# cr1m5onk1ng/text_similarity

Hardware: AMD Instinct MI355X
Metric: sentences/sec encoded + Mpairs/sec cosine top-k @ N=1M d=384 (higher is better)
Workload: dtype bf16 encoder / f16 selection / fp32 scores

## Files before the change

text_similarity_amd/csrc/encoder.hip:

```cpp
#include <math.h>
#include <cmath>

#include <stdlib.h>
#include <string.h>

#include <vector>

#include <type_traits>
#include <utility>

#include "common.h"
#include "gemm_pp.h"

namespace tsim {

__device__ __forceinline__ int64_t packed_off(int64_t t, int f, int W) {
    return ((t >> 5) * (W >> 3) + (f >> 3)) * 256 + (t & 31) * 8 + (f & 7);
}

template <int VPL, bool TYPED = false>
__global__ __launch_bounds__(256) void embed_ln_kernel(const int32_t *__restrict__ ids,
                                                       const int32_t *__restrict__ pos,
                                                       const float *__restrict__ word,
                                                       const float *__restrict__ pos_emb,
// ... 1108 lines not shown
    if (wt) {
        const int i = lane & 15, g = lane >> 4;
        const int ntt = (d_out + 15) >> 4;
        const float *xp = x + (int64_t)min(r0 + i, B - 1) * d_in + 4 * g;
        const float *wp[NT];
#pragma unroll
        for (int t = 0; t < NT; ++t) wp[t] = wt + (int64_t)min((wv + DN_WAVES * t) * 16 + i, d_out - 1) * d_in + 4 * g;
        f32x4 acc[NT];
#pragma unroll
        for (int t = 0; t < NT; ++t) acc[t] = f32x4{0.f, 0.f, 0.f, 0.f};
        float4 a = load4_or_zero(xp, 4 * g < d_in), bw[NT];
#pragma unroll
        for (int t = 0; t < NT; ++t) bw[t] = load4_or_zero(wp[t], wv + DN_WAVES * t < ntt && 4 * g < d_in);
        for (int k0 = 0; k0 < d_in; k0 += 16) {
            const int k1 = k0 + 16;
            const bool kin = k1 + 4 * g < d_in;
            const float4 an = load4_or_zero(xp + k1, kin);
            float4 bn[NT];
#pragma unroll
            for (int t = 0; t < NT; ++t) bn[t] = load4_or_zero(wp[t] + k1, wv + DN_WAVES * t < ntt && kin);
#pragma unroll
            for (int t = 0; t < NT; ++t) {
                if (wv + DN_WAVES * t < ntt) {
                    acc[t] = __builtin_amdgcn_mfma_f32_16x16x4f32(a.x, bw[t].x, acc[t], 0, 0, 0);
                    acc[t] = __builtin_amdgcn_mfma_f32_16x16x4f32(a.y, bw[t].y, acc[t], 0, 0, 0);
                    acc[t] = __builtin_amdgcn_mfma_f32_16x16x4f32(a.z, bw[t].z, acc[t], 0, 0, 0);
                    acc[t] = __builtin_amdgcn_mfma_f32_16x16x4f32(a.w, bw[t].w, acc[t], 0, 0, 0);
                }
            }
            a = an;
#pragma unroll
            for (int t = 0; t < NT; ++t) bw[t] = bn[t];
        }
#pragma unroll
        for (int t = 0; t < NT; ++t) {
            const int col = (wv + DN_WAVES * t) * 16 + i;
            if (col < d_out) {
#pragma unroll
                for (int r = 0; r < 4; ++r) ys[(4 * g + r) * d_out + col] = acc[t][r];
            }
        }
    } else {
        for (int k = threadIdx.x; k < DN_ROWS * d_out; k += 64 * DN_WAVES) {
            const int r = k / d_out;
            ys[k] = r0 + r < B ? x[(int64_t)(r0 + r) * d_in + (k - r * d_out)] : 0.f;
        }
    }
    __syncthreads();
    for (int r = wv; r < DN_ROWS; r += DN_WAVES) {
        const int b = r0 + r;
        if (b >= B) break;
        float *y = ys + r * d_out;
        for (int j = lane; j < d_out; j += 64) {
            float v = y[j];
            if (bias) v += bias[j];
            if (act == TSIM_ACT_TANH) v = tanhf(v);
            y[j] = v;
        }
        if (normalize) {
            double ss = 0.0;
            for (int j = lane; j < d_out; j += 64) ss = fma((double)y[j], (double)y[j], ss);
            const double inv = canonical_inv_norm(ss, 1e-12f);
            for (int j = lane; j < d_out; j += 64) y[j] = canonical_scale_f32(y[j], inv);
        }
        if (out)
            for (int j = lane; j < d_out; j += 64) out[(int64_t)b * d_out + j] = y[j];
        if (unit) {
            double ss = 0.0;
            for (int j = lane; j < d_out; j += 64) ss = fma((double)y[j], (double)y[j], ss);
            const double inv = canonical_inv_norm(ss, 1e-8f);
            double r2 = 0.0;
            for (int j = lane; j < ld_unit; j += 64) {
                unit_t hv = (unit_t)0;
                if (j < d_out) {
                    hv = canonical_unit_elem(y[j], inv);
                    const double de = (double)(float)hv - (double)y[j] * inv;
                    r2 = fma(de, de, r2);
                }
                unit[(int64_t)b * ld_unit + j] = hv;
            }
            if (rho_max) {
                const float rho = rho_round_up(sqrt(wave_sum_f64(r2)));
                if (lane == 0) rho_publish(rho_max, rho);
            }
        }
    }
}

static int dense_rows_launch(const float *x, int B, int d_in, const float *w, const float *bias, int d_out, int act, int normalize,
                             float *out, unit_t *unit, int ld_unit, float *rho_max, hipStream_t st) {
    if (B <= 0) return TSIM_OK;
    const dim3 grid((unsigned)((B + DN_ROWS - 1) / DN_ROWS));
    const size_t lds = (size_t)DN_ROWS * d_out * sizeof(float);
#define DENSE(NT) hipLaunchKernelGGL(dense_rows_kernel<NT>, grid, dim3(64 * DN_WAVES), lds, st, x, B, d_in, w, bias, d_out, act, normalize, out, unit, ld_unit, rho_max)
    const int nt = ((d_out + 15) / 16 + DN_WAVES - 1) / DN_WAVES;
    if (nt <= 1) DENSE(1); else if (nt <= 2) DENSE(2); else if (nt <= 3) DENSE(3); else if (nt <= 4) DENSE(4);
    else if (nt <= 6) DENSE(6); else DENSE(8);
#undef DENSE
    TSIM_HIP_CHECK(hipGetLastError());
    return TSIM_OK;
}

static int dense_check(int d_in, int d_out, int act, const float *w) {
    TSIM_REQUIRE(d_in >= 8 && d_in <= DN_MAX && d_in % 8 == 0, "dense: d_in=%d outside [8, %d] or not a multiple of 8", d_in, DN_MAX);
    TSIM_REQUIRE(d_out >= 8 && d_out <= DN_MAX && d_out % 8 == 0, "dense: d_out=%d outside [8, %d] or not a multiple of 8", d_out,
                 DN_MAX);
    TSIM_REQUIRE(w || d_out == d_in, "dense: without a weight matrix d_out (%d) must equal d_in (%d)", d_out, d_in);
    TSIM_REQUIRE(act == TSIM_ACT_IDENTITY || act == TSIM_ACT_TANH, "dense: unknown activation %d (TSIM_ACT_IDENTITY, TSIM_ACT_TANH)",
                 act);
    TSIM_REQUIRE(((uintptr_t)w & 15) == 0, "dense: the weight matrix must be 16-byte aligned");
    return TSIM_OK;
}

static uint16_t host_f32_to_bf16(float f) {
    uint32_t u;
    memcpy(&u, &f, 4);
    if ((u & 0x7fffffffu) > 0x7f800000u) return (uint16_t)((u >> 16) | 0x40);
    u += 0x7fffu + ((u >> 16) & 1u);
    return (uint16_t)(u >> 16);
}

struct DevBuf {
    void *p = nullptr;
    ~DevBuf() {
        if (p) (void)hipFree(p);
    }
};

}

using namespace tsim;

struct tsim_encoder {
    tsim_encoder_config cfg;
    int Tp = 0;
    float *word = nullptr, *pos = nullptr, *type0 = nullptr, *emb_g = nullptr, *emb_b = nullptr, *relb = nullptr;
    int relw = 0;
    int n_types = 0;
    float *head_wpT = nullptr, *head_bp = nullptr, *head_wc = nullptr, *head_bc = nullptr;
    int n_labels = 0;
    struct Layer {
        bf16_t *wqkv, *wo, *w1, *w2;
        bf16_t *pqkv = nullptr, *po = nullptr;
        bf16_t *lo = nullptr, *l2 = nullptr;
        bf16_t *lo32 = nullptr, *l232 = nullptr;
        uint8_t *qqkv = nullptr, *qo = nullptr, *q1 = nullptr, *q2 = nullptr;
        uint8_t *sqkv = nullptr, *so = nullptr, *s1 = nullptr, *s2 = nullptr;
        float *bqkv, *bo, *b1, *b2, *g1, *be1, *g2, *be2;
    };
    std::vector<Layer> layers;
    std::vector<void *> allocs;
    bf16_t *x0 = nullptr, *x1 = nullptr, *qkv = nullptr, *ctx = nullptr, *h1 = nullptr;
    float *ybuf = nullptr;
    float *head_x = nullptr;
    uint8_t *aq = nullptr, *as = nullptr, *hq = nullptr, *hs = nullptr;
    int *err_flags = nullptr;
};

namespace tsim {

static int dev_alloc(tsim_encoder *e, size_t bytes, void **out) {
    void *p = nullptr;
    hipError_t err = hipMalloc(&p, bytes);
    if (err != hipSuccess) return fail(TSIM_ENOMEM, "hipMalloc(%zu) failed: %s", bytes, hipGetErrorString(err));
    e->allocs.push_back(p);
    *out = p;
    return TSIM_OK;
}

static int upload_f32(tsim_encoder *e, const float *h, size_t n, float **out) {
    int rc = dev_alloc(e, n * 4, (void **)out);
    if (rc) return rc;
    TSIM_HIP_CHECK(hipMemcpy(*out, h, n * 4, hipMemcpyHostToDevice));
    return TSIM_OK;
}

static int upload_bf16(tsim_encoder *e, const std::vector<const float *> &parts, size_t n_each, bf16_t **out) {
    std::vector<uint16_t> tmp(n_each * parts.size());
    for (size_t p = 0; p < parts.size(); ++p)
        for (size_t i = 0; i < n_each; ++i) tmp[p * n_each + i] = host_f32_to_bf16(parts[p][i]);
    int rc = dev_alloc(e, tmp.size() * 2, (void **)out);
    if (rc) return rc;
    TSIM_HIP_CHECK(hipMemcpy(*out, tmp.data(), tmp.size() * 2, hipMemcpyHostToDevice));
    return TSIM_OK;
}

static uint8_t host_f32_to_e4m3(float v) {
    const uint8_t sign = std::signbit(v) ? 0x80 : 0;
    const double a = std::fabs((double)v);
    if (a == 0.0) return sign;
    int exp;
    const double mant = std::frexp(a, &exp);
    long byte;
    if (a >= std::ldexp(1.0, -6))
        byte = ((long)(exp - 1 + 7) << 3) + std::lrint((mant * 2.0 - 1.0) * 8.0);
    else
        byte = std::lrint(std::ldexp(a, 9));
    if (byte > 0x7e) byte = 0x7e;
    return (uint8_t)byte | sign;
}

static int upload_mxfp8(tsim_encoder *e, const std::vector<const float *> &parts, size_t n_rows, size_t K, uint8_t **q,
                        uint8_t **sc) {
    const size_t rows = n_rows * parts.size(), nb = K / 32;
    std::vector<uint8_t> hq(rows * K), hs(rows * nb);
    for (size_t p = 0; p < parts.size(); ++p)
        for (size_t r = 0; r < n_rows; ++r)
            for (size_t b = 0; b < nb; ++b) {
                const float *src = parts[p] + r * K + b * 32;
                float amax = 0.f;
                for (int i = 0; i < 32; ++i) amax = std::fmax(amax, std::fabs(src[i]));
                int sexp = 0;
                if (amax > 0.f) {
                    int ex;
                    (void)std::frexp((double)amax, &ex);
                    sexp = ex - 1 - 8;
                    sexp = sexp < -127 ? -127 : (sexp > 127 ? 127 : sexp);
                }
                uint8_t *dst = hq.data() + (p * n_rows + r) * K + b * 32;
                for (int i = 0; i < 32; ++i) {
                    double y = std::ldexp((double)src[i], -sexp);
                    y = y > 448.0 ? 448.0 : (y < -448.0 ? -448.0 : y);
                    dst[i] = host_f32_to_e4m3((float)y);
                }
                hs[(p * n_rows + r) * nb + b] = (uint8_t)(sexp + 127);
            }
    int rc = dev_alloc(e, hq.size(), (void **)q);
    if (rc) return rc;
    if ((rc = dev_alloc(e, hs.size(), (void **)sc))) return rc;
    TSIM_HIP_CHECK(hipMemcpy(*q, hq.data(), hq.size(), hipMemcpyHostToDevice));
    TSIM_HIP_CHECK(hipMemcpy(*sc, hs.data(), hs.size(), hipMemcpyHostToDevice));
    return TSIM_OK;
}

static int mpnet_bucket(int rel, int num_buckets) {
    int ret = 0;
    int n = -rel;
    const int nb = num_buckets / 2;
    if (n < 0) {
        ret += nb;
        n = -n;
    }
    const int max_exact = nb / 2;
    if (n < max_exact) return ret + n;
    const float v = logf((float)n / (float)max_exact) / (float)log(128.0 / max_exact) * (float)(nb - max_exact);
    int large = max_exact + (int)v;
    if (large > nb - 1) large = nb - 1;
    return ret + large;
}

template <int BM, int BN, int BK, int WM, int WN, int EPI, int NST = 2>
static int launch_gemm(const bf16_t *X, const bf16_t *W, const float *bias, const bf16_t *res, const float *gamma,
                       const float *beta, float eps, bf16_t *out, int M, int N, int K, hipStream_t st,
                       const bf16_t *Wimg = nullptr, bool xpacked = false) {
    constexpr int lds = gemm_lds_bytes<BM, BN, BK, WM, WN, NST>();
    static_assert(lds <= 160 * 1024, "LDS budget");
    auto kern = gemm_bf16_kernel<BM, BN, BK, WM, WN, EPI, NST>;
    static DevOnce lds_once;
    TSIM_MAX_LDS(lds_once, kern, lds);
    if (N % BN != 0 || K % BK != 0) return fail(TSIM_EUNSUPPORTED, "gemm: N=%d K=%d not tileable by %dx%d", N, K, BN, BK);
    const int mtiles = (M + BM - 1) / BM, ntiles = N / BN;
    const int grid = ((mtiles + 7) / 8) * 8 * ntiles;
    if (Wimg && ntiles != 1) return fail(TSIM_EINVAL, "gemm: a packed W image needs BN == N");
    hipLaunchKernelGGL(kern, dim3(grid), dim3(WM * WN * 64), lds, st, X, W, bias, res, gamma, beta, eps, out, M, N, K,
                       mtiles, ntiles, Wimg, xpacked ? 1 : 0);
    TSIM_HIP_CHECK(hipGetLastError());
    return TSIM_OK;
}

template <int EPI, bool PK>
static int gemm_xres2(const bf16_t *X, const bf16_t *W, const float *bias, bf16_t *out, int M, int N, hipStream_t st) {
    constexpr int lds = X2_NSTAGE * X2_BN * X2_BK * 2 + 8192;
    if (N > 2048) return fail(TSIM_EUNSUPPORTED, "gemm_xres2: N=%d > 2048", N);
    if (((int64_t)M + 256) * N * 2 >= (1ll << 32)) return fail(TSIM_EUNSUPPORTED, "gemm_xres2: output of %d x %d exceeds 4 GiB", M, N);
    auto kern = gemm_xres2_kernel<EPI, PK>;
    static DevOnce lds_once;
    TSIM_MAX_LDS(lds_once, kern, lds);
    const int items = ((M + 255) / 256) * (N / X2_BN);
    const int grid = items < 256 ? items : 256;
    hipLaunchKernelGGL(kern, dim3(grid), dim3(512), lds, st, X, W, bias, out, M, N, items);
    TSIM_HIP_CHECK(hipGetLastError());
    return TSIM_OK;
}

typedef __attribute__((ext_vector_type(4))) uint32_t lt_u32x4;
constexpr int LT_PF = 12;
template <int PF>
__global__ __launch_bounds__(256) __attribute__((amdgpu_waves_per_eu(1, 1))) void ln_tail_gemm_kernel(
    const bf16_t *__restrict__ X, const bf16_t *__restrict__ Wimg32, const float *__restrict__ bias, const bf16_t *__restrict__ res,
    const float *__restrict__ gamma, const float *__restrict__ beta, float eps, bf16_t *__restrict__ out, int M, int K, int xpacked) {
    constexpr int N = 384, NT = 3, WAVES_N = 4, BM = 32;
    __shared__ float red[2 * WAVES_N * BM];
    const int lane = threadIdx.x & 63;
    const int wn = __builtin_amdgcn_readfirstlane(threadIdx.x >> 6);
    const int r = lane & 31, h = lane >> 5;
    const int m0 = blockIdx.x * BM;
    const int ksteps = K / 16;

    const int64_t mrow = (int64_t)(m0 + r < M ? m0 + r : M - 1);
    const char *xp = reinterpret_cast<const char *>(X) +
                     (xpacked ? (int64_t)(m0 >> 5) * K * 64 + h * 512 + r * 16
                              : (mrow * K + 8 * h) * 2);
    const int xstep = xpacked ? 1024 : 32;
    const char *wp = reinterpret_cast<const char *>(Wimg32) + (int64_t)(NT * wn) * 1024 + lane * 16;
    constexpr int WSTEP = (N / 32) * 1024;

    f32x16 acc[NT];
#pragma unroll
    for (int i = 0; i < NT; ++i)
#pragma unroll
        for (int gq = 0; gq < 4; ++gq) {
            const float4 bv = *reinterpret_cast<const float4 *>(bias + wn * 96 + 4 * h + i * 32 + 8 * gq);
            acc[i][4 * gq + 0] = bv.x;
            acc[i][4 * gq + 1] = bv.y;
            acc[i][4 * gq + 2] = bv.z;
            acc[i][4 * gq + 3] = bv.w;
        }
#pragma unroll
    for (int i = 0; i < NT; ++i) asm volatile("" : "+v"(acc[i]));

    lt_u32x4 fw[PF][NT], fx[PF];
    auto issue = [&](auto slotc, int s) __attribute__((always_inline)) {
        constexpr int slot = decltype(slotc)::value;
        const int sc = s < ksteps ? s : ksteps - 1;
        const char *w = wp + (int64_t)sc * WSTEP;
        const char *x = xp + (int64_t)sc * xstep;
        lt_u32x4 &f0 = fw[slot][0], &f1 = fw[slot][1], &f2 = fw[slot][2], &f3 = fx[slot];
        asm volatile("global_load_dwordx4 %0, %1, off" : "=v"(f0) : "v"(w) : "memory");
        asm volatile("global_load_dwordx4 %0, %1, off offset:1024" : "=v"(f1) : "v"(w) : "memory");
        asm volatile("global_load_dwordx4 %0, %1, off offset:2048" : "=v"(f2) : "v"(w) : "memory");
        asm volatile("global_load_dwordx4 %0, %1, off" : "=v"(f3) : "v"(x) : "memory");
    };
    ff_static_for(std::make_integer_sequence<int, PF>{}, [&](auto sc) __attribute__((always_inline)) { issue(sc, decltype(sc)::value); });
    for (int s0 = 0; s0 < ksteps; s0 += PF) {
        ff_static_for(std::make_integer_sequence<int, PF>{}, [&](auto sc) __attribute__((always_inline)) {
            constexpr int slot = decltype(sc)::value;
            lt_u32x4 &f0 = fw[slot][0], &f1 = fw[slot][1], &f2 = fw[slot][2], &f3 = fx[slot];
            asm volatile("s_waitcnt vmcnt(%4)" : "+v"(f0), "+v"(f1), "+v"(f2), "+v"(f3) : "n"(4 * (PF - 1)) : "memory");
            const bf16x8 bx = __builtin_bit_cast(bf16x8, f3);
            acc[0] = __builtin_amdgcn_mfma_f32_32x32x16_bf16(__builtin_bit_cast(bf16x8, f0), bx, acc[0], 0, 0, 0);
            acc[1] = __builtin_amdgcn_mfma_f32_32x32x16_bf16(__builtin_bit_cast(bf16x8, f1), bx, acc[1], 0, 0, 0);
            acc[2] = __builtin_amdgcn_mfma_f32_32x32x16_bf16(__builtin_bit_cast(bf16x8, f2), bx, acc[2], 0, 0, 0);
            asm volatile("" : "+v"(f0), "+v"(f1), "+v"(f2), "+v"(f3));
            issue(sc, s0 + slot + PF);
        });
    }
    wait_vmcnt<0>();

    const int nbase = wn * 96 + 4 * h;
    {
        const int64_t m = m0 + r;
        const int64_t mr = m < M ? m : M - 1;
#pragma unroll
        for (int i = 0; i < NT; ++i)
#pragma unroll
            for (int gq = 0; gq < 4; gq += 2) {
                const uint4 o = *reinterpret_cast<const uint4 *>(res + mr * N + wn * 96 + i * 32 + 8 * gq + 8 * h);
                auto s0 = __builtin_amdgcn_permlane32_swap(o.x, o.z, false, false);
                auto s1 = __builtin_amdgcn_permlane32_swap(o.y, o.w, false, false);
                const uint32_t a0 = s0[0], c0 = s0[1], a1 = s1[0], c1 = s1[1];
                acc[i][4 * gq + 0] += __uint_as_float(a0 << 16);
                acc[i][4 * gq + 1] += __uint_as_float(a0 & 0xffff0000u);
                acc[i][4 * gq + 2] += __uint_as_float(a1 << 16);
                acc[i][4 * gq + 3] += __uint_as_float(a1 & 0xffff0000u);
                acc[i][4 * gq + 4] += __uint_as_float(c0 << 16);
                acc[i][4 * gq + 5] += __uint_as_float(c0 & 0xffff0000u);
                acc[i][4 * gq + 6] += __uint_as_float(c1 << 16);
                acc[i][4 * gq + 7] += __uint_as_float(c1 & 0xffff0000u);
            }
    }
    float mean = 0.f, rstd = 0.f;
#pragma unroll
    for (int pass = 0; pass < 2; ++pass) {
        float s = 0.f;
#pragma unroll
        for (int i = 0; i < NT; ++i)
#pragma unroll
            for (int g = 0; g < 16; ++g) {
                if (pass == 0) {
                    s += acc[i][g];
                } else {
                    const float dlt = acc[i][g] - mean;
                    s = fmaf(dlt, dlt, s);
                }
            }
        s += __shfl_xor(s, 32, 64);
        if (h == 0) red[(pass * WAVES_N + wn) * BM + r] = s;
        __syncthreads();
        float t = 0.f;
#pragma unroll
        for (int w = 0; w < WAVES_N; ++w) t += red[(pass * WAVES_N + w) * BM + r];
        if (pass == 0)
            mean = t / (float)N;
        else
            rstd = 1.0f / sqrtf(t / (float)N + eps);
    }
#pragma unroll
    for (int i = 0; i < NT; ++i) {
        float4 gv[4], be[4];
#pragma unroll
        for (int gq = 0; gq < 4; ++gq) {
            gv[gq] = *reinterpret_cast<const float4 *>(gamma + nbase + i * 32 + 8 * gq);
            be[gq] = *reinterpret_cast<const float4 *>(beta + nbase + i * 32 + 8 * gq);
        }
        uint32_t pk[8];
#pragma unroll
        for (int gq = 0; gq < 4; ++gq) {
            const float y0 = fmaf((acc[i][4 * gq + 0] - mean) * rstd, gv[gq].x, be[gq].x);
            const float y1 = fmaf((acc[i][4 * gq + 1] - mean) * rstd, gv[gq].y, be[gq].y);
            const float y2 = fmaf((acc[i][4 * gq + 2] - mean) * rstd, gv[gq].z, be[gq].z);
            const float y3 = fmaf((acc[i][4 * gq + 3] - mean) * rstd, gv[gq].w, be[gq].w);
            pk[2 * gq] = pack_bf16x2(y0, y1);
            pk[2 * gq + 1] = pack_bf16x2(y2, y3);
        }
        const int64_t m = m0 + r;
#pragma unroll
        for (int gq = 0; gq < 4; gq += 2) {
            auto s0 = __builtin_amdgcn_permlane32_swap(pk[2 * gq], pk[2 * gq + 2], false, false);
            auto s1 = __builtin_amdgcn_permlane32_swap(pk[2 * gq + 1], pk[2 * gq + 3], false, false);
            if (m < M)
                *reinterpret_cast<uint4 *>(out + m * N + wn * 96 + i * 32 + 8 * gq + 8 * h) = make_uint4(s0[0], s1[0], s0[1], s1[1]);
        }
    }
}

static int ln_tail_gemm(const bf16_t *X, const bf16_t *Wimg32, const float *bias, const bf16_t *res, const float *gamma,
                        const float *beta, float eps, bf16_t *out, int M, int K, hipStream_t st, bool xpacked) {
    if (K % (16 * LT_PF) != 0) return fail(TSIM_EUNSUPPORTED, "ln_tail_gemm: K=%d", K);
    hipLaunchKernelGGL(ln_tail_gemm_kernel<LT_PF>, dim3((unsigned)((M + 31) / 32)), dim3(256), 0, st, X, Wimg32, bias, res, gamma, beta,
                       eps, out, M, K, xpacked ? 1 : 0);
    TSIM_HIP_CHECK(hipGetLastError());
    return TSIM_OK;
}

template <int NW, int NST>
static int ln_rows_gemm(const bf16_t *X, const bf16_t *Wimg32, const float *bias, const bf16_t *res, const float *gamma,
                        const float *beta, float eps, bf16_t *out, int M, int K, hipStream_t st, bool xpacked) {
    constexpr int lds = NST * (NW * 32 * LR_BK * 2 + LR_WBYTES);
    static_assert(lds <= 160 * 1024, "LDS budget");
    auto kern = ln_rows_gemm_kernel<NW, NST>;
    static DevOnce lds_once;
    TSIM_MAX_LDS(lds_once, kern, lds);
    if (K % LR_BK != 0 || K < NST * LR_BK) return fail(TSIM_EUNSUPPORTED, "ln_rows_gemm: K=%d", K);
    hipLaunchKernelGGL(kern, dim3((unsigned)((M + NW * 32 - 1) / (NW * 32))), dim3(NW * 64), lds, st, X, Wimg32, bias, res, gamma,
                       beta, eps, out, M, K, xpacked ? 1 : 0);
    TSIM_HIP_CHECK(hipGetLastError());
    return TSIM_OK;
}

static bool use_packed_layout(int H, int F) {
    return H == 384 && (3 * H) % X2_BN == 0 && F % X2_BN == 0 && F <= 2048;
}

template <int EPI>
static int gemm_plain(const bf16_t *X, const bf16_t *W, const bf16_t *Wp, const float *bias, bf16_t *out, int M, int N,
                      int K, hipStream_t st) {
    if (K == 384 && N % XR_BN == 0) return gemm_xres2<EPI, false>(X, W, bias, out, M, N, st);
    if (K >= 768 && gemm_pp_supported(N, K))
        return gemm_pp(EPI == EPI_GELU ? PP_EPI_GELU : PP_EPI_BIAS, X, Wp ? Wp : W, Wp != nullptr, bias, out, M, N, K, st);
    if (N % 128 == 0)
        return launch_gemm<128, 128, 64, 2, 2, EPI>(X, W, bias, nullptr, nullptr, nullptr, 0.f, out, M, N, K, st);
    return launch_gemm<128, 64, 64, 2, 2, EPI>(X, W, bias, nullptr, nullptr, nullptr, 0.f, out, M, N, K, st);
}

static int gemm_res_ln(const bf16_t *X, const bf16_t *W, const bf16_t *Wp, const float *bias, const bf16_t *res,
                       const float *gamma, const float *beta, float eps, bf16_t *out, int M, int N, int K, float *ybuf,
                       hipStream_t st, const bf16_t *Wimg = nullptr, const bf16_t *Wimg32 = nullptr, bool xpacked = false) {
    if (xpacked && N != 384) return fail(TSIM_EINVAL, "gemm_res_ln: the packed operand layout is a hidden-384 form");
    if (ybuf && N >= 512 && N % 256 == 0 && gemm_pp_supported(N, K)) {
        int rc = gemm_pp(PP_EPI_F32, X, Wp ? Wp : W, Wp != nullptr, bias, ybuf, M, N, K, st);
        if (rc) return rc;
        return res_ln_rows(ybuf, res, gamma, beta, eps, out, nullptr, nullptr, M, N, st);
    }
    switch (N) {
        case 384: {
            bool after_rows = false;
            if (Wimg32) {
                const int t256 = M / 256;
                const int use = (t256 % 256) >= 128 ? t256 : (t256 / 256) * 256;
                if (use > 0) {
                    int rc = ln_rows_gemm<8, 3>(X, Wimg32, bias, res, gamma, beta, eps, out, use * 256, K, st, xpacked);
                    const int m1 = use * 256;
                    if (rc || m1 == M) return rc;
                    X += (int64_t)m1 * K; res += (int64_t)m1 * N; out += (int64_t)m1 * N; M -= m1;
                    after_rows = true;
                }
                if (M <= 256 * 32 && K % (16 * LT_PF) == 0)
                    return ln_tail_gemm(X, Wimg32, bias, res, gamma, beta, eps, out, M, K, st, xpacked);
            }
            const int mt = (M + 127) / 128, full = (mt / 256) * 256, rem = mt - full;
            auto main_launch = [&](int rows) {
                return launch_gemm<128, 384, 64, 2, 4, EPI_RES_LN>(X, W, bias, res, gamma, beta, eps, out, rows, N, K, st, Wimg, xpacked);
            };
            if (rem > 0 && rem <= 96 && (full > 0 || after_rows)) {
                const int m_main = full * 128;
                if (full > 0) {
                    int rc = main_launch(m_main);
                    if (rc) return rc;
                }
                return launch_gemm<64, 384, 64, 2, 4, EPI_RES_LN>(X + (int64_t)m_main * K, W, bias, res + (int64_t)m_main * N,
                                                                  gamma, beta, eps, out + (int64_t)m_main * N, M - m_main, N, K, st, Wimg, xpacked);
            }
            return main_launch(M);
        }
        case 768: return launch_gemm<64, 768, 32, 1, 8, EPI_RES_LN>(X, W, bias, res, gamma, beta, eps, out, M, N, K, st);
        case 64: return launch_gemm<128, 64, 64, 4, 2, EPI_RES_LN>(X, W, bias, res, gamma, beta, eps, out, M, N, K, st);
        default: return fail(TSIM_EUNSUPPORTED, "encoder: hidden size %d has no fused LayerNorm GEMM (64, 384, 768)", N);
    }
}

}

extern "C" int tsim_encoder_create(const tsim_encoder_config *cfg, const tsim_encoder_weights_host *w,
                                   tsim_encoder **out) {
    TSIM_REQUIRE(cfg && w && out, "encoder_create: null pointer");
    const int H = cfg->hidden, F = cfg->ffn, L = cfg->num_layers;
    TSIM_REQUIRE(H == 64 || H == 384 || H == 768, "encoder_create: hidden=%d unsupported (64, 384, 768)", H);
    TSIM_REQUIRE(cfg->heads > 0 && H % cfg->heads == 0, "encoder_create: heads=%d does not divide hidden=%d", cfg->heads, H);
    const int dh = H / cfg->heads;
    TSIM_REQUIRE(dh == 16 || dh == 32 || dh == 64, "encoder_create: head_dim=%d unsupported (16, 32, 64)", dh);
    TSIM_REQUIRE(F % 64 == 0 && L > 0 && cfg->max_tokens > 0 && cfg->max_seqs > 0, "encoder_create: bad ffn/layers/capacity");
    TSIM_REQUIRE(cfg->arch == TSIM_ARCH_BERT || cfg->arch == TSIM_ARCH_MPNET, "encoder_create: unknown arch");
    TSIM_REQUIRE(w->word_emb && w->pos_emb && w->emb_ln_g && w->emb_ln_b && w->layers, "encoder_create: missing weights");
    TSIM_REQUIRE(cfg->arch != TSIM_ARCH_MPNET || w->rel_bias, "encoder_create: MPNet needs rel_bias");
    const bool mx = cfg->weight_dtype == TSIM_W_MXFP8;
    TSIM_REQUIRE(cfg->weight_dtype == TSIM_W_BF16 || mx, "encoder_create: unknown weight_dtype %d", cfg->weight_dtype);
    if (mx && !(gemm_pp_mx_supported(H, H) && gemm_pp_mx_supported(3 * H, H) && gemm_pp_mx_supported(F, H) && gemm_pp_mx_supported(H, F)))
        return fail(TSIM_EUNSUPPORTED, "encoder_create: MXFP8 projections need hidden and ffn to be multiples of 256 (got %d, %d)", H, F);
    tsim_encoder *e = new tsim_encoder();
    e->cfg = *cfg;
    e->Tp = (cfg->max_tokens + 127) / 128 * 128 + 128;
    int rc = TSIM_OK;
    auto bail = [&](int code) {
        tsim_encoder_destroy(e);
        return code;
    };
    if ((rc = upload_f32(e, w->word_emb, (size_t)cfg->vocab * H, &e->word))) return bail(rc);
    if ((rc = upload_f32(e, w->pos_emb, (size_t)cfg->max_pos * H, &e->pos))) return bail(rc);
    if (w->type_emb && (rc = upload_f32(e, w->type_emb, H, &e->type0))) return bail(rc);
    if ((rc = upload_f32(e, w->emb_ln_g, H, &e->emb_g))) return bail(rc);
    if ((rc = upload_f32(e, w->emb_ln_b, H, &e->emb_b))) return bail(rc);
    if (cfg->arch == TSIM_ARCH_MPNET) {
        const int maxp = cfg->max_pos;
        e->relw = 2 * maxp - 1;
        std::vector<float> tab((size_t)cfg->heads * e->relw);
        for (int d = -(maxp - 1); d <= maxp - 1; ++d) {
            const int bk = mpnet_bucket(d, cfg->rel_buckets);
            for (int hh = 0; hh < cfg->heads; ++hh) tab[(size_t)hh * e->relw + d + maxp - 1] = w->rel_bias[bk * cfg->heads + hh];
        }
        if ((rc = upload_f32(e, tab.data(), tab.size(), &e->relb))) return bail(rc);
    }
    e->layers.resize(L);
    for (int l = 0; l < L; ++l) {
        const tsim_layer_weights_host &lw = w->layers[l];
        tsim_encoder::Layer &d = e->layers[l];
        if ((rc = upload_bf16(e, {lw.wq, lw.wk, lw.wv}, (size_t)H * H, &d.wqkv))) return bail(rc);
        if ((rc = upload_bf16(e, {lw.wo}, (size_t)H * H, &d.wo))) return bail(rc);
        if ((rc = upload_bf16(e, {lw.w1}, (size_t)F * H, &d.w1))) return bail(rc);
        if ((rc = upload_bf16(e, {lw.w2}, (size_t)H * F, &d.w2))) return bail(rc);
        if (mx) {
            if ((rc = upload_mxfp8(e, {lw.wq, lw.wk, lw.wv}, H, H, &d.qqkv, &d.sqkv))) return bail(rc);
            if ((rc = upload_mxfp8(e, {lw.wo}, H, H, &d.qo, &d.so))) return bail(rc);
            if ((rc = upload_mxfp8(e, {lw.w1}, F, H, &d.q1, &d.s1))) return bail(rc);
            if ((rc = upload_mxfp8(e, {lw.w2}, H, F, &d.q2, &d.s2))) return bail(rc);
        }
        auto repack = [&](const void *src, int n_rows, int kbytes, void **dst) {
            int r2 = dev_alloc(e, (size_t)n_rows * kbytes, dst);
            return r2 ? r2 : pack_w(src, *dst, n_rows, kbytes, gemm_pp_tile_width(n_rows), nullptr);
        };
        if (mx) {
            void *t;
            if ((rc = repack(d.qqkv, 3 * H, H, &t))) return bail(rc); d.qqkv = (uint8_t *)t;
            if ((rc = repack(d.qo, H, H, &t))) return bail(rc); d.qo = (uint8_t *)t;
            if ((rc = repack(d.q1, F, H, &t))) return bail(rc); d.q1 = (uint8_t *)t;
            if ((rc = repack(d.q2, H, F, &t))) return bail(rc); d.q2 = (uint8_t *)t;
        } else if (H >= 512 && H % 256 == 0 && gemm_pp_supported(H, H) && gemm_pp_supported(F, H) && gemm_pp_supported(H, F)) {
            if ((rc = repack(d.wqkv, 3 * H, H * 2, (void **)&d.pqkv))) return bail(rc);
            if ((rc = repack(d.wo, H, H * 2, (void **)&d.po))) return bail(rc);
        }
        if (!mx && H == 384 && F % 64 == 0) {
            if ((rc = dev_alloc(e, (size_t)H * H * 2, (void **)&d.lo))) return bail(rc);
            if ((rc = dev_alloc(e, (size_t)H * F * 2, (void **)&d.l2))) return bail(rc);
            hipLaunchKernelGGL(pack_gemm_w_kernel, dim3((unsigned)((H * H / 8 + 255) / 256)), dim3(256), 0, 0,
                               reinterpret_cast<const uint4 *>(d.wo), reinterpret_cast<uint4 *>(d.lo), 384, 64, H);
            hipLaunchKernelGGL(pack_gemm_w_kernel, dim3((unsigned)((H * F / 8 + 255) / 256)), dim3(256), 0, 0,
                               reinterpret_cast<const uint4 *>(d.w2), reinterpret_cast<uint4 *>(d.l2), 384, 64, F);
            if ((rc = dev_alloc(e, (size_t)H * H * 2, (void **)&d.lo32))) return bail(rc);
            if ((rc = dev_alloc(e, (size_t)H * F * 2, (void **)&d.l232))) return bail(rc);
            hipLaunchKernelGGL(pack_frag_w_kernel, dim3((unsigned)((H * H / 8 + 255) / 256)), dim3(256), 0, 0,
                               reinterpret_cast<const uint4 *>(d.wo), reinterpret_cast<uint4 *>(d.lo32), 384, H);
            hipLaunchKernelGGL(pack_frag_w_kernel, dim3((unsigned)((H * F / 8 + 255) / 256)), dim3(256), 0, 0,
                               reinterpret_cast<const uint4 *>(d.w2), reinterpret_cast<uint4 *>(d.l232), 384, F);
            if (hipGetLastError() != hipSuccess) return bail(fail(TSIM_EHIP, "LayerNorm GEMM weight packing failed"));
        }
        std::vector<float> bq(3 * (size_t)H);
        memcpy(bq.data(), lw.bq, H * 4);
        memcpy(bq.data() + H, lw.bk, H * 4);
        memcpy(bq.data() + 2 * H, lw.bv, H * 4);
        if ((rc = upload_f32(e, bq.data(), bq.size(), &d.bqkv))) return bail(rc);
        if ((rc = upload_f32(e, lw.bo, H, &d.bo))) return bail(rc);
        if ((rc = upload_f32(e, lw.b1, F, &d.b1))) return bail(rc);
        if ((rc = upload_f32(e, lw.b2, H, &d.b2))) return bail(rc);
        if ((rc = upload_f32(e, lw.ln1_g, H, &d.g1))) return bail(rc);
        if ((rc = upload_f32(e, lw.ln1_b, H, &d.be1))) return bail(rc);
        if ((rc = upload_f32(e, lw.ln2_g, H, &d.g2))) return bail(rc);
        if ((rc = upload_f32(e, lw.ln2_b, H, &d.be2))) return bail(rc);
    }
    const size_t Tp = e->Tp;
    struct { bf16_t **p; size_t n; } acts[] = {{&e->x0, Tp * H}, {&e->x1, Tp * H}, {&e->qkv, Tp * 3 * H},
                                               {&e->ctx, Tp * H}, {&e->h1, Tp * F}};
    for (auto &a : acts) {
        if ((rc = dev_alloc(e, a.n * 2, (void **)a.p))) return bail(rc);
        if (hipMemset(*a.p, 0, a.n * 2) != hipSuccess) return bail(fail(TSIM_EHIP, "hipMemset failed"));
    }
    if (H >= 512 && H % 256 == 0 && gemm_pp_supported(H, H)) {
        if ((rc = dev_alloc(e, Tp * H * 4, (void **)&e->ybuf))) return bail(rc);
        if (hipMemset(e->ybuf, 0, Tp * H * 4) != hipSuccess) return bail(fail(TSIM_EHIP, "hipMemset failed"));
    }
    if ((size_t)cfg->max_seqs * H * 4 > Tp * 3 * H * 2 && (rc = dev_alloc(e, (size_t)cfg->max_seqs * H * 4, (void **)&e->head_x)))
        return bail(rc);
    if (mx) {
        struct { uint8_t **p; size_t n; } qb[] = {{&e->aq, Tp * H}, {&e->as, Tp * H / 32}, {&e->hq, Tp * F}, {&e->hs, Tp * F / 32}};
        for (auto &a : qb) {
            if ((rc = dev_alloc(e, a.n, (void **)a.p))) return bail(rc);
            if (hipMemset(*a.p, 0, a.n) != hipSuccess) return bail(fail(TSIM_EHIP, "hipMemset failed"));
        }
    }
    if ((rc = dev_alloc(e, 256, (void **)&e->err_flags))) return bail(rc);
    if (hipMemset(e->err_flags, 0, 256) != hipSuccess) return bail(fail(TSIM_EHIP, "hipMemset failed"));
    if (hipDeviceSynchronize() != hipSuccess) return bail(fail(TSIM_EHIP, "sync after upload failed"));
    *out = e;
    return TSIM_OK;
}

extern "C" int tsim_encoder_error_flags(tsim_encoder *e, int32_t *flags_host, void *stream) {
    TSIM_REQUIRE(e && flags_host, "encoder_error_flags: null pointer");
    hipStream_t st = reinterpret_cast<hipStream_t>(stream);
    TSIM_HIP_CHECK(hipMemcpyAsync(flags_host, e->err_flags, 4, hipMemcpyDeviceToHost, st));
    TSIM_HIP_CHECK(hipMemsetAsync(e->err_flags, 0, 4, st));
    TSIM_HIP_CHECK(hipStreamSynchronize(st));
    return TSIM_OK;
}

extern "C" int tsim_quantize_mxfp8(const void *x_bf16, int64_t rows, int K, void *q_out, void *scale_out, void *stream) {
    TSIM_REQUIRE(x_bf16 && q_out && scale_out, "quantize_mxfp8: null pointer");
    TSIM_REQUIRE(rows >= 0 && K > 0, "quantize_mxfp8: bad shape rows=%lld K=%d", (long long)rows, K);
    return quant_mx(static_cast<const bf16_t *>(x_bf16), rows, K, static_cast<uint8_t *>(q_out),
                    static_cast<uint8_t *>(scale_out), reinterpret_cast<hipStream_t>(stream));
}

extern "C" int tsim_gemm_mxfp8(const void *xq, const void *xs, const void *wq, const void *ws, const float *bias,
                               float *out_f32, int M, int N, int K, void *stream) {
    TSIM_REQUIRE(xq && xs && wq && ws && bias && out_f32, "gemm_mxfp8: null pointer");
    TSIM_REQUIRE(M >= 0 && N > 0 && K > 0, "gemm_mxfp8: bad shape M=%d N=%d K=%d", M, N, K);
    return gemm_pp_mx(PP_EPI_F32, static_cast<const uint8_t *>(xq), static_cast<const uint8_t *>(xs),
                      static_cast<const uint8_t *>(wq), 0, static_cast<const uint8_t *>(ws), bias, out_f32, nullptr, M, N, K,
                      reinterpret_cast<hipStream_t>(stream));
}

#ifdef TSIM_PP_STAMPS
extern "C" int tsim_debug_xr_stamps(unsigned long long *out8, int reset) {
    if (hipMemcpyFromSymbol(out8, HIP_SYMBOL(tsim::g_xr_stamps), 64) != hipSuccess) return 1;
    if (reset) { unsigned long long z[8] = {0}; if (hipMemcpyToSymbol(HIP_SYMBOL(tsim::g_xr_stamps), z, 64) != hipSuccess) return 1; }
    return 0;
}
#endif

extern "C" void tsim_encoder_destroy(tsim_encoder *e) {
    if (!e) return;
    for (void *p : e->allocs) (void)hipFree(p);
    delete e;
}

extern "C" int tsim_encoder_set_token_types(tsim_encoder *e, const float *type_emb_host, int32_t n_types) {
    TSIM_REQUIRE(e && type_emb_host, "encoder_set_token_types: null pointer");
    TSIM_REQUIRE(e->cfg.arch == TSIM_ARCH_BERT, "encoder_set_token_types: BERT only (MPNet has no token-type table)");
    TSIM_REQUIRE(n_types >= 1, "encoder_set_token_types: n_types=%d < 1", n_types);
    float *tab = nullptr;
    if (int rc = upload_f32(e, type_emb_host, (size_t)n_types * e->cfg.hidden, &tab)) return rc;
    e->type0 = tab;
    e->n_types = n_types;
    return TSIM_OK;
}

extern "C" int tsim_encoder_set_cls_head(tsim_encoder *e, const float *pool_w_host, const float *pool_b_host,
                                         const float *cls_w_host, const float *cls_b_host, int32_t num_labels) {
    TSIM_REQUIRE(e && pool_w_host && pool_b_host && cls_w_host && cls_b_host, "encoder_set_cls_head: null pointer");
    TSIM_REQUIRE(e->cfg.arch == TSIM_ARCH_BERT, "encoder_set_cls_head: BERT only");
    TSIM_REQUIRE(num_labels >= 1 && num_labels <= CLS_MAX_LABELS, "encoder_set_cls_head: num_labels=%d outside [1, %d]", num_labels,
                 CLS_MAX_LABELS);
    const int H = e->cfg.hidden;
    TSIM_REQUIRE(H % 64 == 0 && H <= CLS_MAX_H, "encoder_set_cls_head: hidden=%d unsupported", H);
    std::vector<float> wT((size_t)H * H);
    for (int o = 0; o < H; ++o)
        for (int k = 0; k < H; ++k) wT[(size_t)k * H + o] = pool_w_host[(size_t)o * H + k];
    int rc;
    if ((rc = upload_f32(e, wT.data(), wT.size(), &e->head_wpT))) return rc;
    if ((rc = upload_f32(e, pool_b_host, H, &e->head_bp))) return rc;
    if ((rc = upload_f32(e, cls_w_host, (size_t)num_labels * H, &e->head_wc))) return rc;
    if ((rc = upload_f32(e, cls_b_host, num_labels, &e->head_bc))) return rc;
    e->n_labels = num_labels;
    return TSIM_OK;
}

extern "C" int tsim_encoder_forward(tsim_encoder *e, const int32_t *tok_ids, const int32_t *tok_pos,
                                    const int32_t *tok_col, const int32_t *cu_seqlens, int32_t T, int32_t B,
                                    int32_t max_len, float *pooled_f32, void *unit_bf16, int ld_unit, float *unit_rho_max,
                                    void *last_hidden_bf16, void *stream) {
    return tsim_encoder_forward_ex(e, tok_ids, nullptr, tok_pos, tok_col, cu_seqlens, T, B, max_len, pooled_f32, unit_bf16, ld_unit,
                                   unit_rho_max, last_hidden_bf16, nullptr, stream);
}

extern "C" int tsim_encoder_forward_ex(tsim_encoder *e, const int32_t *tok_ids, const int32_t *tok_type, const int32_t *tok_pos,
                                       const int32_t *tok_col, const int32_t *cu_seqlens, int32_t T, int32_t B,
                                       int32_t max_len, float *pooled_f32, void *unit_bf16, int ld_unit, float *unit_rho_max,
                                       void *last_hidden_bf16, float *logits_f32, void *stream) {
    TSIM_REQUIRE(e && cu_seqlens && (T == 0 || (tok_ids && tok_pos)), "encoder_forward: null pointer");
    TSIM_REQUIRE(!tok_type || e->n_types > 0, "encoder_forward: tok_type given but no token-type table was set "
                 "(tsim_encoder_set_token_types)");
    TSIM_REQUIRE(!logits_f32 || e->n_labels > 0, "encoder_forward: logits requested but no classification head was set "
                 "(tsim_encoder_set_cls_head)");
    TSIM_REQUIRE(T >= 0 && B >= 0 && T <= e->cfg.max_tokens && B <= e->cfg.max_seqs,
                 "encoder_forward: T=%d B=%d exceed capacity (%d tokens, %d sequences)", T, B, e->cfg.max_tokens, e->cfg.max_seqs);
    const int pos_span = max_len + (e->cfg.arch == TSIM_ARCH_MPNET ? e->cfg.pad_id + 1 : 0);
    TSIM_REQUIRE(max_len >= 0 && pos_span <= e->cfg.max_pos,
                 "encoder_forward: sequences of %d tokens need position rows up to %d, the table has %d", max_len, pos_span - 1,
                 e->cfg.max_pos);
    TSIM_REQUIRE(!unit_bf16 || ld_unit >= e->cfg.hidden, "encoder_forward: ld_unit < hidden");
    if (B == 0) return TSIM_OK;
    hipStream_t st = reinterpret_cast<hipStream_t>(stream);
    const tsim_encoder_config &c = e->cfg;
    const int H = c.hidden, F = c.ffn, dh = H / c.heads;
    const bool mx = c.weight_dtype == TSIM_W_MXFP8;
    int rc;
    if (T > 0) {
        const unsigned g = (unsigned)((T + 3) / 4);
        const int32_t *colp = tok_col ? tok_col : tok_pos;
        const int col_limit = tok_col || c.arch == TSIM_ARCH_BERT ? max_len : c.max_pos;
#define EMBED(V) hipLaunchKernelGGL(embed_ln_kernel<V>, dim3(g), dim3(256), 0, st, tok_ids, tok_pos, e->word, e->pos, e->type0, e->emb_g, e->emb_b, c.ln_eps, T, H, e->x0, c.vocab, c.max_pos, colp, col_limit, e->err_flags, nullptr, 0)
#define EMBED_T(V) hipLaunchKernelGGL((embed_ln_kernel<V, true>), dim3(g), dim3(256), 0, st, tok_ids, tok_pos, e->word, e->pos, e->type0, e->emb_g, e->emb_b, c.ln_eps, T, H, e->x0, c.vocab, c.max_pos, colp, col_limit, e->err_flags, tok_type, e->n_types)
        if (tok_type) {
            if (H == 64) EMBED_T(1); else if (H == 384) EMBED_T(6); else EMBED_T(12);
        } else if (H == 64) EMBED(1); else if (H == 384) EMBED(6); else EMBED(12);
#undef EMBED_T
#undef EMBED
        TSIM_HIP_CHECK(hipGetLastError());
        const float scale = 1.0f / sqrtf((float)dh);
        const bool rel = c.arch == TSIM_ARCH_MPNET;
        const bool pk = !mx && !rel && use_packed_layout(H, F);
        const int32_t *col = rel ? (tok_col ? tok_col : tok_pos) : nullptr;
        const int qblocks = (max_len + 31) / 32 > 0 ? (max_len + 31) / 32 : 1;
        const dim3 agrid((unsigned)(((B + 7) / 8) * 8), (unsigned)((c.heads + 3) / 4), (unsigned)qblocks);
        for (int l = 0; l < c.num_layers; ++l) {
            const tsim_encoder::Layer &L = e->layers[l];
            if (mx) {
                if (l == 0 && (rc = quant_mx(e->x0, T, H, e->aq, e->as, st))) return rc;
                if ((rc = gemm_pp_mx(PP_EPI_BIAS, e->aq, e->as, L.qqkv, 1, L.sqkv, L.bqkv, e->qkv, nullptr, T, 3 * H, H, st))) return rc;
            } else if (pk) {
                if ((rc = gemm_xres2<EPI_BIAS, true>(e->x0, L.wqkv, L.bqkv, e->qkv, T, 3 * H, st))) return rc;
            } else if ((rc = gemm_plain<EPI_BIAS>(e->x0, L.wqkv, L.pqkv, L.bqkv, e->qkv, T, 3 * H, H, st))) return rc;
#define ATT(D)                                                                                                 \
    do {                                                                                                       \
        if (rel)                                                                                               \
            hipLaunchKernelGGL((attention_kernel<D, true>), agrid, dim3(256), 0, st, e->qkv, cu_seqlens, col,  \
                               e->relb, e->relw, H, c.heads, scale, e->ctx, B, 1);                                         \
        else if (pk)                                                                                           \
            hipLaunchKernelGGL((attention_kernel<D, false, true>), agrid, dim3(256), 0, st, e->qkv, cu_seqlens, col, \
                               e->relb, e->relw, H, c.heads, scale, e->ctx, B, 1);                                         \
        else                                                                                                   \
            hipLaunchKernelGGL((attention_kernel<D, false>), agrid, dim3(256), 0, st, e->qkv, cu_seqlens, col, \
                               e->relb, e->relw, H, c.heads, scale, e->ctx, B, 1);                                         \
    } while (0)
            if (dh == 16) ATT(16); else if (dh == 32) ATT(32); else ATT(64);
#undef ATT
            TSIM_HIP_CHECK(hipGetLastError());
            if (mx) {
                if ((rc = quant_mx(e->ctx, T, H, e->aq, e->as, st))) return rc;
                if ((rc = gemm_pp_mx(PP_EPI_F32, e->aq, e->as, L.qo, 1, L.so, L.bo, e->ybuf, nullptr, T, H, H, st))) return rc;
                if ((rc = res_ln_rows(e->ybuf, e->x0, L.g1, L.be1, c.ln_eps, e->x1, e->aq, e->as, T, H, st))) return rc;
                if ((rc = gemm_pp_mx(PP_EPI_GELU_MX, e->aq, e->as, L.q1, 1, L.s1, L.b1, e->hq, e->hs, T, F, H, st))) return rc;
                if ((rc = gemm_pp_mx(PP_EPI_F32, e->hq, e->hs, L.q2, 1, L.s2, L.b2, e->ybuf, nullptr, T, H, F, st))) return rc;
                if ((rc = res_ln_rows(e->ybuf, e->x1, L.g2, L.be2, c.ln_eps, e->x0, e->aq, e->as, T, H, st))) return rc;
                continue;
            }
            if ((rc = gemm_res_ln(e->ctx, L.wo, L.po, L.bo, e->x0, L.g1, L.be1, c.ln_eps, e->x1, T, H, H, e->ybuf, st, L.lo, L.lo32))) return rc;
            if (pk) {
                if ((rc = gemm_xres2<EPI_GELU, true>(e->x1, L.w1, L.b1, e->h1, T, F, st))) return rc;
            } else if ((rc = gemm_plain<EPI_GELU>(e->x1, L.w1, nullptr, L.b1, e->h1, T, F, H, st))) return rc;
            if ((rc = gemm_res_ln(e->h1, L.w2, nullptr, L.b2, e->x1, L.g2, L.be2, c.ln_eps, e->x0, T, H, F, e->ybuf, st, L.l2, L.l232, pk))) return rc;
        }
        if (last_hidden_bf16)
            TSIM_HIP_CHECK(hipMemcpyAsync(last_hidden_bf16, e->x0, (size_t)T * H * 2, hipMemcpyDeviceToDevice, st));
    }
    if (pooled_f32 || unit_bf16) {
        const unsigned g = (unsigned)((B + 3) / 4);
#define POOL(V) hipLaunchKernelGGL(pool_packed_kernel<V>, dim3(g), dim3(256), 0, st, e->x0, cu_seqlens, B, H, pooled_f32, (unit_t *)unit_bf16, ld_unit, unit_bf16 ? unit_rho_max : nullptr)
        if (H % 8 != 0 || H > 1024 || (unit_bf16 && ld_unit % 8 != 0))
            return fail(TSIM_EUNSUPPORTED, "encoder: pooling needs a hidden size that is a multiple of 8, at most 1024 (got %d)", H);
        if (((uintptr_t)pooled_f32 | (uintptr_t)unit_bf16) & 15)
            return fail(TSIM_EINVAL, "encoder: pooled / unit outputs must be 16-byte aligned");
        if (H <= 512) POOL(1); else POOL(2);
#undef POOL
        TSIM_HIP_CHECK(hipGetLastError());
    }
    if (logits_f32) {
        hipLaunchKernelGGL(cls_head_kernel, dim3((unsigned)((B + CLS_ROWS - 1) / CLS_ROWS)), dim3((unsigned)H), 0, st, e->x0, cu_seqlens,
                           B, H, e->head_wpT, e->head_bp, e->head_wc, e->head_bc, e->n_labels, logits_f32);
        TSIM_HIP_CHECK(hipGetLastError());
    }
    return TSIM_OK;
}

extern "C" int tsim_encoder_forward_head(tsim_encoder *e, const int32_t *tok_ids, const int32_t *tok_type, const int32_t *tok_pos,
                                         const int32_t *tok_col, const int32_t *cu_seqlens, int32_t T, int32_t B, int32_t max_len,
                                         const tsim_sentence_head *head, float *emb_f32, void *unit_f16, int ld_unit,
                                         float *unit_rho_max, void *last_hidden_bf16, void *stream) {
    if (!head)
        return tsim_encoder_forward_ex(e, tok_ids, tok_type, tok_pos, tok_col, cu_seqlens, T, B, max_len, emb_f32, unit_f16, ld_unit,
                                       unit_rho_max, last_hidden_bf16, nullptr, stream);
    TSIM_REQUIRE(e, "encoder_forward_head: null encoder");
    const int H = e->cfg.hidden, mode = head->pool_mode, d_out = head->d_out;
    TSIM_REQUIRE(mode >= TSIM_POOL_MEAN && mode <= TSIM_POOL_MEAN_SQRT_LEN, "encoder_forward_head: unknown pool_mode %d", mode);
    TSIM_REQUIRE(head->normalize == 0 || head->normalize == 1, "encoder_forward_head: normalize=%d is not 0 / 1", head->normalize);
    TSIM_REQUIRE(d_out >= 0, "encoder_forward_head: d_out=%d < 0", d_out);
    if (d_out) {
        TSIM_REQUIRE(head->dense_w, "encoder_forward_head: d_out=%d without dense_w", d_out);
        if (int rc = dense_check(H, d_out, head->dense_act, head->dense_w)) return rc;
    } else {
        TSIM_REQUIRE(!head->dense_w && !head->dense_b, "encoder_forward_head: dense weights given with d_out = 0");
    }
    const int width = d_out ? d_out : H;
    TSIM_REQUIRE(!unit_f16 || width <= 768, "encoder_forward_head: unit rows need a final width <= 768 (got %d)", width);
    TSIM_REQUIRE(!unit_f16 || (ld_unit >= width && ld_unit % 8 == 0), "encoder_forward_head: ld_unit=%d (final width %d)", ld_unit,
                 width);
    TSIM_REQUIRE(H % 8 == 0 && H <= 1024, "encoder_forward_head: pooling needs hidden %% 8 == 0 and <= 1024 (got %d)", H);
    TSIM_REQUIRE((((uintptr_t)emb_f32 | (uintptr_t)unit_f16) & 15) == 0, "encoder_forward_head: outputs must be 16-byte aligned");
    if (int rc = tsim_encoder_forward_ex(e, tok_ids, tok_type, tok_pos, tok_col, cu_seqlens, T, B, max_len, nullptr, nullptr, 0,
                                         nullptr, last_hidden_bf16, nullptr, stream))
        return rc;
    if (B == 0 || (!emb_f32 && !unit_f16)) return TSIM_OK;
    hipStream_t st = reinterpret_cast<hipStream_t>(stream);
    float *px = d_out ? (e->head_x ? e->head_x : reinterpret_cast<float *>(e->qkv)) : emb_f32;
    unit_t *pu = d_out ? nullptr : static_cast<unit_t *>(unit_f16);
    const bool norm = !d_out && head->normalize;
    const unsigned g = (unsigned)((B + 3) / 4);
#define POOL(NP, M, N) hipLaunchKernelGGL((pool_packed_kernel<NP, M, N>), dim3(g), dim3(256), 0, st, e->x0, cu_seqlens, B, H, px, pu, ld_unit, pu ? unit_rho_max : nullptr)
#define POOL_NP(M, N) do { if (H <= 512) POOL(1, M, N); else POOL(2, M, N); } while (0)
#define POOL_M(N) do { switch (mode) { case TSIM_POOL_MEAN: POOL_NP(TSIM_POOL_MEAN, N); break; case TSIM_POOL_CLS: POOL_NP(TSIM_POOL_CLS, N); break; \
                                       case TSIM_POOL_MAX: POOL_NP(TSIM_POOL_MAX, N); break; default: POOL_NP(TSIM_POOL_MEAN_SQRT_LEN, N); } } while (0)
    if (norm) POOL_M(true); else POOL_M(false);
#undef POOL_M
#undef POOL_NP
#undef POOL
    TSIM_HIP_CHECK(hipGetLastError());
    if (d_out)
        return dense_rows_launch(px, B, H, head->dense_w, head->dense_b, d_out, head->dense_act, head->normalize, emb_f32,
                                 static_cast<unit_t *>(unit_f16), ld_unit, unit_f16 ? unit_rho_max : nullptr, st);
    return TSIM_OK;
}

extern "C" int tsim_dense_rows(const float *x, int64_t B, int d_in, const float *w, const float *b, int d_out, int act, int normalize,
                               float *out, void *stream) {
    TSIM_REQUIRE(x && out, "dense_rows: null pointer");
    TSIM_REQUIRE(B >= 0 && B <= INT32_MAX - DN_ROWS, "dense_rows: bad row count %lld", (long long)B);
    TSIM_REQUIRE(normalize == 0 || normalize == 1, "dense_rows: normalize=%d is not 0 / 1", normalize);
    if (int rc = dense_check(d_in, d_out, act, w)) return rc;
    TSIM_REQUIRE((((uintptr_t)x | (uintptr_t)out) & 15) == 0, "dense_rows: x and out must be 16-byte aligned");
    return dense_rows_launch(x, (int)B, d_in, w, b, d_out, act, normalize, out, nullptr, 0, nullptr, reinterpret_cast<hipStream_t>(stream));
}
```

Measured before the change: 801,100.

## Split small-M LN-tail GEMM across more blocks with separate layernorm finish kernel

When the LN-tail GEMM has few row blocks (64 or 128 blocks of 32 rows or fewer), the four N-slices of each row block now go to two or four separate blocks instead of one 256-thread block. Each block writes fp32 accumulators to a scratch image, and a second kernel reads them back to apply the residual layernorm. The aim is more parallelism across CUs for small batches or remainder tails. The cost is an extra launch and an fp32 round trip through global memory, plus a new scratch allocation.

```diff
diff --git a/text_similarity_amd/csrc/encoder.hip b/text_similarity_amd/csrc/encoder.hip
--- a/text_similarity_amd/csrc/encoder.hip
+++ b/text_similarity_amd/csrc/encoder.hip
@@ -1284,6 +1284,7 @@
     std::vector<void *> allocs;
     bf16_t *x0 = nullptr, *x1 = nullptr, *qkv = nullptr, *ctx = nullptr, *h1 = nullptr;
     float *ybuf = nullptr;
+    float *lnimg = nullptr;
     float *head_x = nullptr;
     uint8_t *aq = nullptr, *as = nullptr, *hq = nullptr, *hs = nullptr;
     int *err_flags = nullptr;
@@ -1417,16 +1418,14 @@
 
 typedef __attribute__((ext_vector_type(4))) uint32_t lt_u32x4;
 constexpr int LT_PF = 12;
+
 template <int PF>
-__global__ __launch_bounds__(256) __attribute__((amdgpu_waves_per_eu(1, 1))) void ln_tail_gemm_kernel(
-    const bf16_t *__restrict__ X, const bf16_t *__restrict__ Wimg32, const float *__restrict__ bias, const bf16_t *__restrict__ res,
-    const float *__restrict__ gamma, const float *__restrict__ beta, float eps, bf16_t *__restrict__ out, int M, int K, int xpacked) {
-    constexpr int N = 384, NT = 3, WAVES_N = 4, BM = 32;
-    __shared__ float red[2 * WAVES_N * BM];
+__device__ __forceinline__ void lt_gemm_slice(const bf16_t *__restrict__ X, const bf16_t *__restrict__ Wimg32,
+                                              const float *__restrict__ bias, const bf16_t *__restrict__ res, int M, int K,
+                                              int xpacked, int wn, int m0, f32x16 (&acc)[3]) {
+    constexpr int N = 384, NT = 3;
     const int lane = threadIdx.x & 63;
-    const int wn = __builtin_amdgcn_readfirstlane(threadIdx.x >> 6);
     const int r = lane & 31, h = lane >> 5;
-    const int m0 = blockIdx.x * BM;
     const int ksteps = K / 16;
 
     const int64_t mrow = (int64_t)(m0 + r < M ? m0 + r : M - 1);
@@ -1437,7 +1436,6 @@
     const char *wp = reinterpret_cast<const char *>(Wimg32) + (int64_t)(NT * wn) * 1024 + lane * 16;
     constexpr int WSTEP = (N / 32) * 1024;
 
-    f32x16 acc[NT];
 #pragma unroll
     for (int i = 0; i < NT; ++i)
 #pragma unroll
@@ -1479,7 +1477,6 @@
     }
     wait_vmcnt<0>();
 
-    const int nbase = wn * 96 + 4 * h;
     {
         const int64_t m = m0 + r;
         const int64_t mr = m < M ? m : M - 1;
@@ -1501,6 +1498,15 @@
                 acc[i][4 * gq + 7] += __uint_as_float(c1 & 0xffff0000u);
             }
     }
+}
+
+__device__ __forceinline__ void lt_layernorm(f32x16 (&acc)[3], float *red, const float *__restrict__ gamma,
+                                             const float *__restrict__ beta, float eps, bf16_t *__restrict__ out, int M, int wn,
+                                             int m0) {
+    constexpr int N = 384, NT = 3, WAVES_N = 4, BM = 32;
+    const int lane = threadIdx.x & 63;
+    const int r = lane & 31, h = lane >> 5;
+    const int nbase = wn * 96 + 4 * h;
     float mean = 0.f, rstd = 0.f;
 #pragma unroll
     for (int pass = 0; pass < 2; ++pass) {
@@ -1556,11 +1562,78 @@
     }
 }
 
+template <int PF>
+__global__ __launch_bounds__(256) __attribute__((amdgpu_waves_per_eu(1, 1))) void ln_tail_gemm_kernel(
+    const bf16_t *__restrict__ X, const bf16_t *__restrict__ Wimg32, const float *__restrict__ bias, const bf16_t *__restrict__ res,
+    const float *__restrict__ gamma, const float *__restrict__ beta, float eps, bf16_t *__restrict__ out, int M, int K, int xpacked) {
+    __shared__ float red[2 * 4 * 32];
+    const int wn = __builtin_amdgcn_readfirstlane(threadIdx.x >> 6);
+    const int m0 = blockIdx.x * 32;
+    f32x16 acc[3];
+    lt_gemm_slice<PF>(X, Wimg32, bias, res, M, K, xpacked, wn, m0, acc);
+    lt_layernorm(acc, red, gamma, beta, eps, out, M, wn, m0);
+}
+
+constexpr int LS_MAX_BLOCKS = 256;
+
+template <int PF, int S>
+__global__ __launch_bounds__(256 / S) __attribute__((amdgpu_waves_per_eu(1, 1))) void ln_split_gemm_kernel(
+    const bf16_t *__restrict__ X, const bf16_t *__restrict__ Wimg32, const float *__restrict__ bias, const bf16_t *__restrict__ res,
+    float4 *__restrict__ img, int M, int K, int xpacked) {
+    const int blk = blockIdx.x / S, sl = blockIdx.x % S;
+    const int wn = __builtin_amdgcn_readfirstlane(sl * (4 / S) + (threadIdx.x >> 6));
+    const int m0 = blk * 32;
+    f32x16 acc[3];
+    lt_gemm_slice<PF>(X, Wimg32, bias, res, M, K, xpacked, wn, m0, acc);
+    float4 *dst = img + (int64_t)(blk * 4 + wn) * 12 * 64 + (threadIdx.x & 63);
+#pragma unroll
+    for (int i = 0; i < 3; ++i)
+#pragma unroll
+        for (int gq = 0; gq < 4; ++gq)
+            dst[(i * 4 + gq) * 64] = make_float4(acc[i][4 * gq + 0], acc[i][4 * gq + 1], acc[i][4 * gq + 2], acc[i][4 * gq + 3]);
+}
+
+__global__ __launch_bounds__(256) void ln_split_finish_kernel(const float4 *__restrict__ img, const float *__restrict__ gamma,
+                                                              const float *__restrict__ beta, float eps, bf16_t *__restrict__ out,
+                                                              int M) {
+    __shared__ float red[2 * 4 * 32];
+    const int wn = __builtin_amdgcn_readfirstlane(threadIdx.x >> 6);
+    const int m0 = blockIdx.x * 32;
+    const float4 *src = img + (int64_t)(blockIdx.x * 4 + wn) * 12 * 64 + (threadIdx.x & 63);
+    f32x16 acc[3];
+#pragma unroll
+    for (int i = 0; i < 3; ++i)
+#pragma unroll
+        for (int gq = 0; gq < 4; ++gq) {
+            const float4 v = src[(i * 4 + gq) * 64];
+            acc[i][4 * gq + 0] = v.x;
+            acc[i][4 * gq + 1] = v.y;
+            acc[i][4 * gq + 2] = v.z;
+            acc[i][4 * gq + 3] = v.w;
+        }
+    lt_layernorm(acc, red, gamma, beta, eps, out, M, wn, m0);
+}
+
 static int ln_tail_gemm(const bf16_t *X, const bf16_t *Wimg32, const float *bias, const bf16_t *res, const float *gamma,
-                        const float *beta, float eps, bf16_t *out, int M, int K, hipStream_t st, bool xpacked) {
+                        const float *beta, float eps, bf16_t *out, int M, int K, hipStream_t st, bool xpacked, float *img) {
     if (K % (16 * LT_PF) != 0) return fail(TSIM_EUNSUPPORTED, "ln_tail_gemm: K=%d", K);
-    hipLaunchKernelGGL(ln_tail_gemm_kernel<LT_PF>, dim3((unsigned)((M + 31) / 32)), dim3(256), 0, st, X, Wimg32, bias, res, gamma, beta,
-                       eps, out, M, K, xpacked ? 1 : 0);
+    const int nb = (M + 31) / 32;
+    const int S = !img || nb > LS_MAX_BLOCKS ? 1 : nb <= 64 ? 4 : nb <= 128 ? 2 : 1;
+    if (S == 1) {
+        hipLaunchKernelGGL(ln_tail_gemm_kernel<LT_PF>, dim3((unsigned)nb), dim3(256), 0, st, X, Wimg32, bias, res, gamma, beta, eps,
+                           out, M, K, xpacked ? 1 : 0);
+        TSIM_HIP_CHECK(hipGetLastError());
+        return TSIM_OK;
+    }
+    float4 *im = reinterpret_cast<float4 *>(img);
+    if (S == 4)
+        hipLaunchKernelGGL((ln_split_gemm_kernel<LT_PF, 4>), dim3((unsigned)(nb * 4)), dim3(64), 0, st, X, Wimg32, bias, res, im, M, K,
+                           xpacked ? 1 : 0);
+    else
+        hipLaunchKernelGGL((ln_split_gemm_kernel<LT_PF, 2>), dim3((unsigned)(nb * 2)), dim3(128), 0, st, X, Wimg32, bias, res, im, M,
+                           K, xpacked ? 1 : 0);
+    TSIM_HIP_CHECK(hipGetLastError());
+    hipLaunchKernelGGL(ln_split_finish_kernel, dim3((unsigned)nb), dim3(256), 0, st, im, gamma, beta, eps, out, M);
     TSIM_HIP_CHECK(hipGetLastError());
     return TSIM_OK;
 }
@@ -1597,7 +1670,8 @@
 
 static int gemm_res_ln(const bf16_t *X, const bf16_t *W, const bf16_t *Wp, const float *bias, const bf16_t *res,
                        const float *gamma, const float *beta, float eps, bf16_t *out, int M, int N, int K, float *ybuf,
-                       hipStream_t st, const bf16_t *Wimg = nullptr, const bf16_t *Wimg32 = nullptr, bool xpacked = false) {
+                       hipStream_t st, const bf16_t *Wimg = nullptr, const bf16_t *Wimg32 = nullptr, bool xpacked = false,
+                       float *lnimg = nullptr) {
     if (xpacked && N != 384) return fail(TSIM_EINVAL, "gemm_res_ln: the packed operand layout is a hidden-384 form");
     if (ybuf && N >= 512 && N % 256 == 0 && gemm_pp_supported(N, K)) {
         int rc = gemm_pp(PP_EPI_F32, X, Wp ? Wp : W, Wp != nullptr, bias, ybuf, M, N, K, st);
@@ -1617,8 +1691,8 @@
                     X += (int64_t)m1 * K; res += (int64_t)m1 * N; out += (int64_t)m1 * N; M -= m1;
                     after_rows = true;
                 }
-                if (M <= 256 * 32 && K % (16 * LT_PF) == 0)
-                    return ln_tail_gemm(X, Wimg32, bias, res, gamma, beta, eps, out, M, K, st, xpacked);
+                if (M <= LS_MAX_BLOCKS * 32 && K % (16 * LT_PF) == 0)
+                    return ln_tail_gemm(X, Wimg32, bias, res, gamma, beta, eps, out, M, K, st, xpacked, lnimg);
             }
             const int mt = (M + 127) / 128, full = (mt / 256) * 256, rem = mt - full;
             auto main_launch = [&](int rows) {
@@ -1748,6 +1822,12 @@
     if (H >= 512 && H % 256 == 0 && gemm_pp_supported(H, H)) {
         if ((rc = dev_alloc(e, Tp * H * 4, (void **)&e->ybuf))) return bail(rc);
         if (hipMemset(e->ybuf, 0, Tp * H * 4) != hipSuccess) return bail(fail(TSIM_EHIP, "hipMemset failed"));
+    }
+    if (!mx && H == 384 && F % 64 == 0) {
+        const size_t blocks = (Tp + 31) / 32 < (size_t)LS_MAX_BLOCKS ? (Tp + 31) / 32 : (size_t)LS_MAX_BLOCKS;
+        const size_t bytes = blocks * 4 * 12 * 64 * 16;
+        if ((rc = dev_alloc(e, bytes, (void **)&e->lnimg))) return bail(rc);
+        if (hipMemset(e->lnimg, 0, bytes) != hipSuccess) return bail(fail(TSIM_EHIP, "hipMemset failed"));
     }
     if ((size_t)cfg->max_seqs * H * 4 > Tp * 3 * H * 2 && (rc = dev_alloc(e, (size_t)cfg->max_seqs * H * 4, (void **)&e->head_x)))
         return bail(rc);
@@ -1915,11 +1995,11 @@
                 if ((rc = res_ln_rows(e->ybuf, e->x1, L.g2, L.be2, c.ln_eps, e->x0, e->aq, e->as, T, H, st))) return rc;
                 continue;
             }
-            if ((rc = gemm_res_ln(e->ctx, L.wo, L.po, L.bo, e->x0, L.g1, L.be1, c.ln_eps, e->x1, T, H, H, e->ybuf, st, L.lo, L.lo32))) return rc;
+            if ((rc = gemm_res_ln(e->ctx, L.wo, L.po, L.bo, e->x0, L.g1, L.be1, c.ln_eps, e->x1, T, H, H, e->ybuf, st, L.lo, L.lo32, false, e->lnimg))) return rc;
             if (pk) {
                 if ((rc = gemm_xres2<EPI_GELU, true>(e->x1, L.w1, L.b1, e->h1, T, F, st))) return rc;
             } else if ((rc = gemm_plain<EPI_GELU>(e->x1, L.w1, nullptr, L.b1, e->h1, T, F, H, st))) return rc;
-            if ((rc = gemm_res_ln(e->h1, L.w2, nullptr, L.b2, e->x1, L.g2, L.be2, c.ln_eps, e->x0, T, H, F, e->ybuf, st, L.l2, L.l232, pk))) return rc;
+            if ((rc = gemm_res_ln(e->h1, L.w2, nullptr, L.b2, e->x1, L.g2, L.be2, c.ln_eps, e->x0, T, H, F, e->ybuf, st, L.l2, L.l232, pk, e->lnimg))) return rc;
         }
         if (last_hidden_bf16)
             TSIM_HIP_CHECK(hipMemcpyAsync(last_hidden_bf16, e->x0, (size_t)T * H * 2, hipMemcpyDeviceToDevice, st));
```

After: 813,800 (median of 6 runs). 1.02x the previous value.
